# tatary/ramses

Hardware: AMD Instinct MI355X
Metric: cell-updates/s (Godunov sweep), uniform Sedov3D (higher is better)
Workload: dtype f64

## Files before the change

ramses_amd/csrc/hydro_core.hpp:

```cpp
#pragma once
#include <hip/hip_runtime.h>

namespace ramses_amd {

constexpr int RIEMANN_LLF = 0, RIEMANN_HLLC = 1, RIEMANN_HLL = 2,
              RIEMANN_ACOUSTIC = 3, RIEMANN_EXACT = 4;

constexpr int MAX_NENER = 2;
constexpr int MAX_NVAR = 16;

struct HydroConst {
  double gamma;
  double smallr;
  double smallc;
  double smallp;
  double smalle;
  double entho;
  double gm1;
  double smallc2;
  double gamma6;
  double smallpp;
  double oneovergamma;
  double slope_theta;
  int niter_riemann;
// ... 20 lines not shown
  r = __builtin_fma(r, e, r);
#endif
  return r;
}
RA_DEV double ddiv(double a, double b) { return a * rcp_fast(b); }
RA_DEV double dsqrt(double x) {
  double y = __builtin_amdgcn_rsq(x);
  double g = x * y;
  double h = 0.5 * y;
  double r = __builtin_fma(-h, g, 0.5);
  g = __builtin_fma(g, r, g);
  h = __builtin_fma(h, r, h);
  const double d = __builtin_fma(-g, g, x);
  g = __builtin_fma(d, h, g);
  return x == 0.0 ? 0.0 : g;
}
#else
RA_DEV double ddiv(double a, double b) { return a / b; }
RA_DEV double dsqrt(double x) { return __builtin_sqrt(x); }
#endif

template <int NV, bool GRAV, int NE = 0>
RA_DEV void ctoprim_cell(const double (&u)[NV], const double (&g)[3],
                         double dtxhalf, const HydroConst &P, double (&q)[NV]) {
  const double rho = dmaxd(u[0], P.smallr);
  const double oneoverrho = ddiv(1.0, rho);
  const double vx = u[1] * oneoverrho;
  const double vy = u[2] * oneoverrho;
  const double vz = u[3] * oneoverrho;
#ifdef RAMSES_AMD_FAST
  double k2 = vx * vx;
  k2 = __builtin_fma(vy, vy, k2);
  k2 = __builtin_fma(vz, vz, k2);
  double eint;
  if constexpr (NE == 0) {
    eint = dmaxd(__builtin_fma(u[4], oneoverrho, -0.5 * k2), P.smalle);
  } else {
    double erad = u[5] * oneoverrho;
    if constexpr (NE > 1) erad = __builtin_fma(u[6], oneoverrho, erad);
    eint = dmaxd(__builtin_fma(u[4], oneoverrho, -0.5 * k2) - erad, P.smalle);
  }
#else
  double eken = 0.5 * vx * vx;
  eken = eken + 0.5 * vy * vy;
  eken = eken + 0.5 * vz * vz;
  double eint;
  if constexpr (NE == 0) {
    eint = dmaxd(u[4] * oneoverrho - eken, P.smalle);
  } else {
// ... 104 lines not shown
  const double q0 = nb[13];
  double vmin = nb[0] - q0, vmax = vmin;
#pragma unroll
  for (int t = 1; t < 27; t++) {
    const double df = nb[t] - q0;
    vmin = dmind(vmin, df);
    vmax = dmaxd(vmax, df);
  }
  const double dfx = 0.5 * (nb[14] - nb[12]);
  const double dfy = 0.5 * (nb[16] - nb[10]);
  const double dfz = 0.5 * (nb[22] - nb[4]);
  const double dff = 0.5 * (__builtin_fabs(dfx) + __builtin_fabs(dfy) + __builtin_fabs(dfz));
  double slop = 1.0;
  if (dff > 0.0) slop = dmind(1.0, dmind(__builtin_fabs(vmin), __builtin_fabs(vmax)) / dff);
  d[0] = slop * dfx;
  d[1] = slop * dfy;
  d[2] = slop * dfz;
}

template <int NV, int NE = 0>
RA_DEV void trace3d_cell(const double (&q)[NV], const double (&dq)[3][NV],
                         double dtdx, double dtdy, double dtdz,
                         const HydroConst &P, double (&qm)[3][NV],
                         double (&qp)[3][NV]) {
  const double r = q[0], u = q[1], v = q[2], w = q[3], p = q[4];
  const double drx = dq[0][0], dux = dq[0][1], dvx = dq[0][2], dwx = dq[0][3], dpx = dq[0][4];
  const double dry = dq[1][0], duy = dq[1][1], dvy = dq[1][2], dwy = dq[1][3], dpy = dq[1][4];
  const double drz = dq[2][0], duz = dq[2][1], dvz = dq[2][2], dwz = dq[2][3], dpz = dq[2][4];
  const double div = dux + dvy + dwz;
#ifdef RAMSES_AMD_FAST
  const double rinv = rcp_fast(r);
  auto adv = [&](double ax, double ay, double az, double c0, double c1) {
    double t = u * ax;
    t = __builtin_fma(v, ay, t);
    t = __builtin_fma(w, az, t);
    return -__builtin_fma(c0, c1, t);
  };
  const double sr0 = adv(drx, dry, drz, div, r);
  const double sp0 = adv(dpx, dpy, dpz, div * P.gamma, p);
  double su0 = adv(dux, duy, duz, dpx, rinv);
  double sv0 = adv(dvx, dvy, dvz, dpy, rinv);
  double sw0 = adv(dwx, dwy, dwz, dpz, rinv);
  double se0[NE > 0 ? NE : 1];
#pragma unroll
  for (int i = 0; i < NE; i++) {
    su0 = __builtin_fma(-dq[0][5 + i], rinv, su0);
    sv0 = __builtin_fma(-dq[1][5 + i], rinv, sv0);
    sw0 = __builtin_fma(-dq[2][5 + i], rinv, sw0);
    se0[i] = adv(dq[0][5 + i], dq[1][5 + i], dq[2][5 + i], div * P.gamma_rad[i], q[5 + i]);
  }
#else
  const double sr0 = -u * drx - v * dry - w * drz - (div)*r;
  const double sp0 = -u * dpx - v * dpy - w * dpz - (div)*P.gamma * p;
  double su0 = -u * dux - v * duy - w * duz - (dpx) / r;
// ... 490 lines not shown
  a[2] = qL[4]; b[2] = qR[4];
  a[3] = qL[lt1]; b[3] = qR[lt1];
  a[4] = qL[lt2]; b[4] = qR[lt2];
#pragma unroll
  for (int n = 5; n < NV; n++) { a[n] = qL[n]; b[n] = qR[n]; }
  riemann_solve<RS, NV, NE>(a, b, P, f);
  flux[0] = f[0];
  flux[ln] = f[1];
  flux[lt1] = f[3];
  flux[lt2] = f[4];
  flux[4] = f[2];
#pragma unroll
  for (int n = 5; n < NV; n++) flux[n] = f[n];
  unorm = 0.5 * (a[1] + b[1]);
  eflux = f[NV];
}

#ifdef RAMSES_AMD_FAST
RA_DEV double rsqrt_fast(double x) {
  double y = __builtin_amdgcn_rsq(x);
  const double e = __builtin_fma(-(x * y), y, 1.0);
  return __builtin_fma(0.5 * y, e, y);
}
template <int DIR>
RA_DEV void llf_flux_fast(const double (&qL)[5], const double (&qR)[5],
                          const HydroConst &P, double dtdx, double (&flux)[5]) {
  constexpr int ln = DIR == 0 ? 1 : (DIR == 1 ? 2 : 3);
  constexpr int lt1 = DIR == 0 ? 2 : 1;
  constexpr int lt2 = DIR == 2 ? 2 : 3;
  const double rl = dmaxd(qL[0], P.smallr), pl = dmaxd(qL[4], rl * P.smallp);
  const double rr = dmaxd(qR[0], P.smallr), pr = dmaxd(qR[4], rr * P.smallp);
  const double gl = P.gamma * pl, gr = P.gamma * pr;
  const double cl = gl * rsqrt_fast(gl * rl);
  const double cr = gr * rsqrt_fast(gr * rr);
  const double ul = qL[ln], ur = qR[ln];
  const double cmax = dmaxd(__builtin_fabs(ul) + cl, __builtin_fabs(ur) + cr);
  const double hs = 0.5 * dtdx;
  const double hc = cmax * hs;
  const double mL = qL[0] * ul, mR = qR[0] * ur;
  double kL = ul * ul; kL = __builtin_fma(qL[lt1], qL[lt1], kL); kL = __builtin_fma(qL[lt2], qL[lt2], kL);
  double kR = ur * ur; kR = __builtin_fma(qR[lt1], qR[lt1], kR); kR = __builtin_fma(qR[lt2], qR[lt2], kR);
  const double eL = __builtin_fma(0.5 * qL[0], kL, qL[4] * P.entho);
  const double eR = __builtin_fma(0.5 * qR[0], kR, qR[4] * P.entho);
  const double t1L = qL[0] * qL[lt1], t1R = qR[0] * qR[lt1];
  const double t2L = qL[0] * qL[lt2], t2R = qR[0] * qR[lt2];
  const double fnL = __builtin_fma(ul, mL, qL[4]), fnR = __builtin_fma(ur, mR, qR[4]);
  const double feR = ur * (eR + qR[4]);
  const double fesum = __builtin_fma(ul, eL + qL[4], feR);
  flux[0] = __builtin_fma(hc, qL[0] - qR[0], hs * (mL + mR));
  flux[ln] = __builtin_fma(hc, mL - mR, hs * (fnL + fnR));
  flux[lt1] = __builtin_fma(hc, t1L - t1R, hs * __builtin_fma(ul, t1L, ur * t1R));
  flux[lt2] = __builtin_fma(hc, t2L - t2R, hs * __builtin_fma(ul, t2L, ur * t2R));
  flux[4] = __builtin_fma(hc, eL - eR, hs * fesum);
}
// ... 19 lines not shown
  const bool star = left ? !(SL > 0.0) : (SR > 0.0);
  const double rk = left ? rl : rr, uk = left ? ul : ur, Pk = left ? Pl : Pr, S = left ? SL : SR;
  const double vl1 = qL[lt1], vr1 = qR[lt1], vl2 = qL[lt2], vr2 = qR[lt2];
  const double w1 = left ? vl1 : vr1, w2 = left ? vl2 : vr2;
  double k2 = uk * uk; k2 = __builtin_fma(w1, w1, k2); k2 = __builtin_fma(w2, w2, k2);
  const double etk = __builtin_fma(0.5 * rk, k2, Pk * P.entho);
  const double inv = rcp_fast(S - ustar);
  const double dS = S - uk;
  const double rst = rk * dS * inv;
  const double ets = __builtin_fma(Pstar, ustar, __builtin_fma(dS, etk, -(Pk * uk))) * inv;
  const double ro = star ? rst : rk, uo = star ? ustar : uk, Po = star ? Pstar : Pk, eto = star ? ets : etk;
  const double m = ro * uo * dtdx;
  flux[0] = m;
  flux[ln] = __builtin_fma(m, uo, Po * dtdx);
  flux[lt1] = m * w1;
  flux[lt2] = m * w2;
  flux[4] = (eto + Po) * (uo * dtdx);
#if RAMSES_AMD_HLLC_FUSED == 2
  __builtin_amdgcn_sched_barrier(0);
#endif
}
#endif

template <int RS, int NV, int DIR, bool FUSE_HLLC = true, int NE = 0>
RA_DEV void scaled_interface_flux(const double (&qL)[NV], const double (&qR)[NV],
                                  const HydroConst &P, double dt, double dx, double rdx,
                                  double dtdx, bool DXPOW2, double (&flux)[NV]) {
#ifdef RAMSES_AMD_FAST
  if constexpr (RS == RIEMANN_LLF && NV == 5) {
    llf_flux_fast<DIR>(qL, qR, P, dtdx, flux);
    return;
  }
#ifndef RAMSES_AMD_HLLC_FUSED
#define RAMSES_AMD_HLLC_FUSED 1
#endif
  if constexpr (RAMSES_AMD_HLLC_FUSED != 0 && FUSE_HLLC && RS == RIEMANN_HLLC && NV == 5) {
    hllc_flux_fast<DIR>(qL, qR, P, dtdx, flux);
    return;
  }
#endif
  double un_, ef_;
  interface_flux<RS, NV, DIR, NE>(qL, qR, P, flux, un_, ef_);
#pragma unroll
  for (int n = 0; n < NV; n++) {
#ifdef RAMSES_AMD_FAST
    flux[n] = flux[n] * dtdx;
#else
    flux[n] = DXPOW2 ? flux[n] * dt * rdx : flux[n] * dt / dx;
#endif
  }
}

template <int RS, int NV, int DIR>
// ... 44 lines not shown
```

ramses_amd/csrc/hydro_sweep.hip:

```cpp
#include <hip/hip_runtime.h>

#include "hydro_core.hpp"
#include "sweep_args.hpp"

namespace ramses_amd {

#ifdef RAMSES_AMD_FAST
#define SWEEP_NS fastmode
#else
#define SWEEP_NS strictmode
#endif

namespace SWEEP_NS {

constexpr int BX = 64;
#ifndef TILE_SWEEP_BY
#define TILE_SWEEP_BY 12
#endif

template <int BY, int NV>
struct Plane {
  double v[NV][BY][BX];
};

template <int ST, int BY, int NV, bool MASK, bool GRAV, int NX = 0>
struct Lds {
  static constexpr int NF = NV + NX;
  static constexpr int RING = (ST == 3) ? 3 : 2;
#ifndef SWEEP_PARK_PLAIN
#ifdef RAMSES_AMD_FAST
#define SWEEP_PARK_PLAIN 1
#else
#define SWEEP_PARK_PLAIN 0
#endif
#endif
  static constexpr bool PARK = MASK || ((GRAV || SWEEP_PARK_PLAIN) && BY == 12);
  static constexpr int MR = PARK ? BY - 2 : BY;
  static constexpr int M0 = PARK ? 1 : 0;
  static constexpr size_t q_off = 0;
  static constexpr size_t m_off = q_off + RING * sizeof(Plane<BY, NV>);
  static constexpr size_t park_off = m_off + 2 * sizeof(Plane<MR, NF>);
  static constexpr size_t mask_off = park_off + (PARK ? sizeof(double) * 2 * NF * (BY - 4) * BX : 0);
  static constexpr size_t sloc_off = mask_off + (MASK ? 3 * BY * BX : 0);
  static constexpr size_t bytes = sloc_off + (MASK ? 4 * BY * BX : 0);
};

__device__ __forceinline__ double wave_shr1(double v) {
  int lo = __double2loint(v), hi = __double2hiint(v);
  lo = __builtin_amdgcn_update_dpp(lo, lo, 0x138, 0xf, 0xf, false);
  hi = __builtin_amdgcn_update_dpp(hi, hi, 0x138, 0xf, 0xf, false);
  return __hiloint2double(hi, lo);
}
__device__ __forceinline__ double wave_shl1(double v) {
  int lo = __double2loint(v), hi = __double2hiint(v);
  lo = __builtin_amdgcn_update_dpp(lo, lo, 0x130, 0xf, 0xf, false);
  hi = __builtin_amdgcn_update_dpp(hi, hi, 0x130, 0xf, 0xf, false);
  return __hiloint2double(hi, lo);
}

enum { ROLE_HALO = 0, ROLE_LOW = 1, ROLE_HIGH = 2, ROLE_FULL = 3, ROLE_HALO_HI = 4 };

typedef unsigned int v2u32 __attribute__((ext_vector_type(2)));
constexpr unsigned BUF_RANGE = 0x7fffffffu;
constexpr unsigned BUF_OOB = 0xffffffffu;
#ifndef SWEEP_STORE_AUX
#define SWEEP_STORE_AUX 0
#endif
__device__ __forceinline__ double plane_load(const double *var_base, unsigned plane_bytes, unsigned off) {
  __amdgpu_buffer_rsrc_t r = __builtin_amdgcn_make_buffer_rsrc(const_cast<double *>(var_base), 0, BUF_RANGE, 0x00020000);
  return __builtin_bit_cast(double, __builtin_amdgcn_raw_buffer_load_b64(r, off, plane_bytes, 0));
}
__device__ __forceinline__ void plane_store(double *var_base, unsigned plane_bytes, unsigned off, double x) {
  __amdgpu_buffer_rsrc_t r = __builtin_amdgcn_make_buffer_rsrc(var_base, 0, BUF_RANGE, 0x00020000);
  __builtin_amdgcn_raw_buffer_store_b64(__builtin_bit_cast(v2u32, x), r, off, plane_bytes, SWEEP_STORE_AUX);
}

__device__ __forceinline__ int wave_shr1_i(int v) { return __builtin_amdgcn_update_dpp(v, v, 0x138, 0xf, 0xf, false); }
__device__ __forceinline__ int wave_shl1_i(int v) { return __builtin_amdgcn_update_dpp(v, v, 0x130, 0xf, 0xf, false); }
__device__ __forceinline__ int stat_load(const unsigned char *base, unsigned ncell, unsigned lane_cell, unsigned plane_cell) {
  __amdgpu_buffer_rsrc_t r = __builtin_amdgcn_make_buffer_rsrc(const_cast<unsigned char *>(base), 0, ncell, 0x00020000);
  return (int)__builtin_amdgcn_raw_buffer_load_b8(r, lane_cell, plane_cell, 0);
}
__device__ __forceinline__ int dir_load(const int *base, unsigned plane_ints, unsigned col) {
  __amdgpu_buffer_rsrc_t r = __builtin_amdgcn_make_buffer_rsrc(const_cast<int *>(base), 0, BUF_RANGE, 0x00020000);
  return (int)__builtin_amdgcn_raw_buffer_load_b32(r, col * 4u, plane_ints * 4u, 0);
}

template <int ST, int RS, int BY, bool GRAV, int SCHEME, int NV, int ROLE, bool MASK, int NE = 0, bool PFIX = false>
__device__ __forceinline__ void sweep_march(const SweepArgs &A, unsigned char *smem_raw, const SweepPfix &X = SweepPfix()) {
  static_assert(!PFIX || (MASK && NE == 0 && SCHEME == 0), "pressure_fix: the sweep of a level in tiles, muscl");
  constexpr int NF = NV + (PFIX ? 2 : 0);
  const bool DXPOW2 = A.pow2 != 0;
  typedef Lds<ST, BY, NV, MASK, GRAV, NF - NV> L;
  constexpr int RING = L::RING;
  constexpr bool PARK = L::PARK;
  constexpr int M0 = L::M0;
  Plane<BY, NV> *qring = reinterpret_cast<Plane<BY, NV> *>(smem_raw + L::q_off);
  Plane<L::MR, NF> *mring = reinterpret_cast<Plane<L::MR, NF> *>(smem_raw + L::m_off);
  double (*park)[BY - 4][BX] = reinterpret_cast<double (*)[BY - 4][BX]>(smem_raw + L::park_off);

  const int tx = threadIdx.x, ty = threadIdx.y;
  const HydroConst &P = A.P;

  const int hb = blockIdx.x;
  int bi = 0;
#pragma unroll
  for (int i = 1; i < 6; i++)
    if (i < A.nbox && hb >= A.box[i].first) bi = i;
  const SweepBox &B = A.box[bi];
  int lb = hb - B.first;
  {
    const int nxcd = 8;
    const int cnt = (bi + 1 < A.nbox ? A.box[bi + 1].first : (int)gridDim.x) - B.first;
    if (cnt % nxcd == 0) {
      const int per = cnt / nxcd;
      lb = (lb % nxcd) * per + lb / nxcd;
    }
  }
#ifndef SWEEP_TILE_YFAST
#define SWEEP_TILE_YFAST 0
#endif
#if SWEEP_TILE_YFAST
// ... 47 lines not shown

#ifndef SWEEP_LATE_BASE
#define SWEEP_LATE_BASE 0
#endif
  constexpr bool LATE = SWEEP_LATE_BASE && NV == 5;
#ifndef SWEEP_KEEP_PLAIN
#define SWEEP_KEEP_PLAIN 1
#endif
#ifndef SWEEP_KEEP_STRICT
#define SWEEP_KEEP_STRICT 0
#endif
#if defined(RAMSES_AMD_FAST) || SWEEP_KEEP_STRICT
#ifndef SWEEP_KEEP_LLF_ONLY
#define SWEEP_KEEP_LLF_ONLY 0
#endif
#ifndef SWEEP_KEEP_NOT_HLLC
#define SWEEP_KEEP_NOT_HLLC 1
#endif
  constexpr bool KEEP = (MASK || (SWEEP_KEEP_PLAIN && BY == 12)) && NV == 5 && !LATE && (!SWEEP_KEEP_LLF_ONLY || RS == RIEMANN_LLF) &&
                        (!SWEEP_KEEP_NOT_HLLC || RS != RIEMANN_HLLC);
#else
  constexpr bool KEEP = false;
#endif
  constexpr bool r_trace = ROLE == ROLE_LOW || ROLE == ROLE_HIGH || ROLE == ROLE_FULL;
  constexpr bool r_fxz = ROLE == ROLE_FULL;
  const bool r_upd = r_fxz && (tx >= 2) && (tx <= BX - 3) && (xu < A.nx) && (yu < A.ny);
  const unsigned colb_upd = r_upd ? colb : BUF_OOB;

  const double dtdx = A.dt / A.dx;
  const double dtxhalf = A.dt * 0.5;

  auto plane_off = [&](int p) -> unsigned {
    int pz;
    if (A.ng == 0) { pz = p < 0 ? p + A.nz : (p >= A.nz ? p - A.nz : p); }
    else { pz = p + A.ng; }
    return (unsigned)pz * (unsigned)(A.pitch_z * 8);
  };
  auto wrap_z = [&](int p) -> int { return p < 0 ? p + A.nz : (p >= A.nz ? p - A.nz : p); };
  constexpr unsigned TILE_VOID = 0x80000000u;
  unsigned sA0 = TILE_VOID, sA1 = TILE_VOID, sB0 = TILE_VOID, sB1 = TILE_VOID;
  auto tile_of_plane = [&](int p) -> int { return wrap_z(p) >> 3; };
  auto tile_set = [&](int tz) {
    typedef const int __attribute__((address_space(4))) *cdir_p;
    const cdir_p row = (cdir_p)(A.dir + (long)tz * (A.ntx * A.nty) + drow);
    const int ra = row[tA], rb = row[tB];
    const unsigned a = ra < 0 ? TILE_VOID : (unsigned)ra * 8u, b = rb < 0 ? TILE_VOID : (unsigned)rb * 8u;
    if (tz & 1) { sA1 = a; sB1 = b; } else { sA0 = a; sB0 = b; }
  };
// ... 21 lines not shown
    if constexpr (PFIX) { u[NV] = plane_load(X.divu, pb, off); u[NV + 1] = plane_load(X.enew, pb, off); }
  };
  int ok_zlo = 0;
  int spre = 0;
  unsigned char *smask = smem_raw + L::mask_off;
  auto load_g = [&](int p, double (&g)[3]) {
    if (GRAV) {
      const unsigned pb = MASK ? zpart(p) * 8u : plane_off(p), off = MASK ? tbp(p) : colb;
#pragma unroll
      for (int d = 0; d < 3; d++) g[d] = plane_load(grav + (long)d * A.pitch_var, pb, off);
    } else {
      g[0] = g[1] = g[2] = 0.0;
    }
  };

  double qmz[NV];
  double fzlo[NF];
  double upre[NV], gpre[3];
  double rold = 0.0, sold[NV > 5 ? NV - 5 : 1];
  double ukeep[NV];
#pragma unroll
  for (int n = 0; n < NV; n++) ukeep[n] = 0.0;

  int sa = 0, sb = 1, sc = 2;

  if (MASK) {
    const int t0 = tile_of_plane(z0 - 2), t1 = t0 + 1 < A.ntz ? t0 + 1 : 0;
    tile_set(t0);
    tile_set(t1);
    __syncthreads();
    if (r_trace) spre = stat_load(A.stat, (unsigned)A.pitch_var, tbp(z0 - 1) >> 3, zpart(z0 - 1));
  }
  {
    double u[NV], g[3], q[NV];
    load_u(z0 - 2, u); load_g(z0 - 2, g);
    ctoprim_cell<NV, GRAV, NE>(u, g, dtxhalf, P, q);
#pragma unroll
    for (int n = 0; n < NV; n++) qring[sa].v[n][ty][tx] = q[n];
    load_u(z0 - 1, u); load_g(z0 - 1, g);
    if (KEEP) {
#pragma unroll
      for (int n = 0; n < NV; n++) ukeep[n] = u[n];
    }
    ctoprim_cell<NV, GRAV, NE>(u, g, dtxhalf, P, q);
#pragma unroll
    for (int n = 0; n < NV; n++) qring[sb].v[n][ty][tx] = q[n];
    load_u(z0, upre); load_g(z0, gpre);
#pragma unroll
    for (int n = 0; n < NV; n++) qmz[n] = 1.0;
#pragma unroll
    for (int n = 0; n < NF; n++) fzlo[n] = 0.0;
  }
  __builtin_amdgcn_s_waitcnt(0x0f70);
  __syncthreads();

  const int txm = tx - 1, txp = tx + 1;
  const int tym = ty - 1, typ = ty + 1;

  double partx[NF];
  double fyown[NF];
  double rnew = 0.0, snew[NV > 5 ? NV - 5 : 1];
  double bcar[NV];
#pragma unroll
  for (int n = 0; n < NV; n++) bcar[n] = 0.0;
#pragma unroll
  for (int n = 0; n < NF; n++) { partx[n] = 0.0; fyown[n] = 0.0; }
  if (PARK && r_fxz) {
#pragma unroll
    for (int n = 0; n < 2 * NF; n++) park[n][ty - 2][tx] = 0.0;
  }

  for (int c = z0 - 1; c <= z1; c++) {
    Plane<L::MR, NF> &M = mring[c & 1];
    Plane<L::MR, NF> &Mprev = mring[(c & 1) ^ 1];
    double qc[NV];
    ctoprim_cell<NV, GRAV, NE>(upre, gpre, dtxhalf, P, qc);
    if (RING == 3 || !r_trace) {
#pragma unroll
      for (int n = 0; n < NV; n++) qring[RING == 3 ? sc : sa].v[n][ty][tx] = qc[n];
    }
    double ucur[NF];
    if (r_fxz && !LATE) {
      if (KEEP && (!MASK || A.base_uold)) {
#pragma unroll
        for (int n = 0; n < NV; n++) ucur[n] = ukeep[n];
      } else if constexpr (MASK) load_base(c, ucur);
      else load_u(c, ucur);
    }
    if (KEEP && r_fxz) {
#pragma unroll
      for (int n = 0; n < NV; n++) ukeep[n] = upre[n];
    }
    int okc = 0, ok_ym = 0;
    if (MASK && r_trace) {
      okc = spre;
      smask[((c + 3) % 3 * BY + ty) * BX + tx] = (unsigned char)okc;
    }

    double qpy[NV], dz[NF], px[NF];
// ... 25 lines not shown
        for (int n = 0; n < NV; n++) qb[n] = qs.v[n][ty][tx];
        const double dc0 = qb[1] * A.dt / A.dx, dc1 = qb[2] * A.dt / A.dx, dc2 = qb[3] * A.dt / A.dx;
#pragma unroll
        for (int n = 0; n < NV; n++) {
          dq[0][n] = slope1_1d<ST>(qs.v[n][ty][txm], qb[n], qs.v[n][ty][txp], dc0, n);
          dq[1][n] = slope1_1d<ST>(qs.v[n][tym][tx], qb[n], qs.v[n][typ][tx], dc1, n);
          dq[2][n] = slope1_1d<ST>(qprev.v[n][ty][tx], qb[n], qc[n], dc2, n);
        }
      } else {
#pragma unroll
        for (int n = 0; n < NV; n++) {
          qb[n] = qs.v[n][ty][tx];
          dq[0][n] = slope1<ST>(qs.v[n][ty][txm], qb[n], qs.v[n][ty][txp], P);
          dq[1][n] = slope1<ST>(qs.v[n][tym][tx], qb[n], qs.v[n][typ][tx], P);
          dq[2][n] = slope1<ST>(qprev.v[n][ty][tx], qb[n], qc[n], P);
        }
      }
      if (RING == 2) {
#pragma unroll
        for (int n = 0; n < NV; n++) qring[sa].v[n][ty][tx] = qc[n];
      }
      double qm[3][NV], qp[3][NV];
      if (SCHEME == 0) {
        trace3d_cell<NV, NE>(qb, dq, dtdx, dtdx, dtdx, P, qm, qp);
      } else {
        const double cc = ctoprim_sound(qb[0], qb[4], P);
        tracexyz_cell<NV>(qb, dq, cc, dtdx, dtdx, dtdx, P, qm, qp);
      }
#pragma unroll
      for (int n = 0; n < NV; n++) M.v[n][ty - M0][tx] = qm[1][n];
#pragma unroll
      for (int n = 0; n < NV; n++) qpy[n] = qp[1][n];
      if constexpr (r_fxz) {
        double qL[NV], fx[NF], fz[NF];
#pragma unroll
        for (int n = 0; n < NV; n++) qL[n] = wave_shr1(qm[0][n]);
        if constexpr (PFIX) {
          double f[NV], t[2];
          scaled_interface_flux_tmp<RS, NV, 0>(qL, qp[0], P, A.dt, A.dx, A.rdx, DXPOW2, f, t);
#pragma unroll
          for (int n = 0; n < NV; n++) fx[n] = f[n];
          fx[NV] = t[0]; fx[NV + 1] = t[1];
          scaled_interface_flux_tmp<RS, NV, 2>(qmz, qp[2], P, A.dt, A.dx, A.rdx, DXPOW2, f, t);
#pragma unroll
          for (int n = 0; n < NV; n++) fz[n] = f[n];
          fz[NV] = t[0]; fz[NV + 1] = t[1];
        } else {
        scaled_interface_flux<RS, NV, 0, !MASK, NE>(qL, qp[0], P, A.dt, A.dx, A.rdx, dtdx, DXPOW2, fx);
        scaled_interface_flux<RS, NV, 2, !MASK, NE>(qmz, qp[2], P, A.dt, A.dx, A.rdx, dtdx, DXPOW2, fz);
        }
        if (MASK) {
          const int s_xm = wave_shr1_i(okc);
          const bool zx = ((okc | s_xm) & CELL_REFINED) != 0, zz = ((okc | ok_zlo) & CELL_REFINED) != 0;
#pragma unroll
          for (int n = 0; n < NF; n++) { fx[n] = zx ? 0.0 : fx[n]; fz[n] = zz ? 0.0 : fz[n]; }
        }
        double fxh[NF];
#pragma unroll
        for (int n = 0; n < NV; n++) qmz[n] = qm[2][n];
#pragma unroll
        for (int n = 0; n < NF; n++) {
          dz[n] = fzlo[n] - fz[n];
          fzlo[n] = fz[n];
          fxh[n] = wave_shl1(fx[n]);
          px[n] = LATE ? (fx[n] - fxh[n]) : ucur[n] + (fx[n] - fxh[n]);
        }
        if (NV > 5 + NE && !MASK) {
          rnew = ucur[0];
#pragma unroll
          for (int n = 5 + NE; n < NV; n++) snew[n - 5] = ucur[n];
        }
      }
    }
    __builtin_amdgcn_sched_barrier(0);
    {
      const int pn = min(c + 2, z1 + 1);
      if (MASK) {
        const int lp = wrap_z(pn) & 7;
        const int tn = tile_of_plane(pn) + 1 < A.ntz ? tile_of_plane(pn) + 1 : 0;
        if (lp == 4) tile_set(tn);
      }
      load_u(pn, upre); load_g(pn, gpre);
      if (MASK && r_trace) { const int ps = min(c + 1, z1 + 1); spre = stat_load(A.stat, (unsigned)A.pitch_var, tbp(ps) >> 3, zpart(ps)); }
    }
    __builtin_amdgcn_sched_barrier(0);
    __syncthreads();

    double fy[NF];
    if constexpr (ROLE == ROLE_FULL || ROLE == ROLE_HIGH) {
      double qL[NV];
#pragma unroll
      for (int n = 0; n < NV; n++) qL[n] = M.v[n][tym - M0][tx];
      if constexpr (PFIX) {
        double f[NV], t[2];
        scaled_interface_flux_tmp<RS, NV, 1>(qL, qpy, P, A.dt, A.dx, A.rdx, DXPOW2, f, t);
#pragma unroll
        for (int n = 0; n < NV; n++) fy[n] = f[n];
        fy[NV] = t[0]; fy[NV + 1] = t[1];
      } else {
      scaled_interface_flux<RS, NV, 1, !MASK, NE>(qL, qpy, P, A.dt, A.dx, A.rdx, dtdx, DXPOW2, fy);
      }
      if (MASK) {
        ok_ym = smask[((c + 3) % 3 * BY + tym) * BX + tx];
        const bool zy = ((okc | ok_ym) & CELL_REFINED) != 0;
#pragma unroll
        for (int n = 0; n < NF; n++) fy[n] = zy ? 0.0 : fy[n];
      }
#pragma unroll
      for (int n = 0; n < NF; n++) M.v[n][tym - M0][tx] = fy[n];
    }
    if constexpr (r_fxz) {
      double un[NF], fyh[NF];
#pragma unroll
      for (int n = 0; n < NF; n++) {
        fyh[n] = Mprev.v[n][ty - M0][tx];
        const double pxn = PARK ? park[n][ty - 2][tx] : partx[n];
        const double fyn = PARK ? park[NF + n][ty - 2][tx] : fyown[n];
        const double part = (LATE ? bcar[n < NV ? n : 0] + pxn : pxn) + (fyn - fyh[n]);
        un[n] = part + dz[n];
      }
      if (NV > 5 + NE && !MASK) {
        if (rold < P.smallr && un[0] > rold) {
#pragma unroll
          for (int n = 5 + NE; n < NV; n++) un[n] = sold[n - 5] * dmaxd(un[0], P.smallr) / P.smallr;
        } else if (un[0] < P.smallr && rold > un[0]) {
#pragma unroll
          for (int n = 5 + NE; n < NV; n++) un[n] = sold[n - 5] * P.smallr / dmaxd(rold, P.smallr);
        }
        rold = rnew;
#pragma unroll
        for (int n = 5 + NE; n < NV; n++) sold[n - 5] = snew[n - 5];
      }
#pragma unroll
      for (int n = 0; n < NF; n++) {
        if (PARK) { park[n][ty - 2][tx] = px[n]; park[NF + n][ty - 2][tx] = fy[n]; }
        else { partx[n] = px[n]; fyown[n] = fy[n]; }
      }
      {
        const unsigned pb = MASK ? zpart(c - 1) * 8u : plane_off(c - 1);
        const unsigned so = (c >= z0 + 1) ? (MASK ? ((r_upd && (ok_zlo & CELL_OWNED)) ? tbp(c - 1) : BUF_OOB) : colb_upd) : BUF_OOB;
#pragma unroll
        for (int n = 0; n < NV; n++) {
          if (MASK) plane_store(unew + (long)(n & ~1) * A.pitch_var, pb + (n & 1) * odd_var, so, un[n]);
          else plane_store(unew + (long)n * A.pitch_var, pb, so, un[n]);
        }
        if constexpr (PFIX) { plane_store(X.divu, pb, so, un[NV]); plane_store(X.enew, pb, so, un[NV + 1]); }
      }
      if constexpr (LATE) { if (MASK) load_base(c, bcar); else load_u(c, bcar); }
    }
    if (RING == 3) { const int t = sa; sa = sb; sb = sc; sc = t; }
    else { const int t = sa; sa = sb; sb = t; }
    if (MASK) ok_zlo = okc;
  }
}

template <int ST, int RS, int BY, bool GRAV, int SCHEME, int NV, bool MASK = false>
__global__ __launch_bounds__(BX *BY) void godunov_sweep_kernel(SweepArgs A) {
  extern __shared__ __attribute__((aligned(16))) unsigned char smem_raw[];
  const int ty = threadIdx.y;
  if (ty >= 2 && ty <= BY - 3) __builtin_amdgcn_s_setprio(3);
  if (ty == 0) sweep_march<ST, RS, BY, GRAV, SCHEME, NV, ROLE_HALO, MASK>(A, smem_raw);
  else if (ty == BY - 1) sweep_march<ST, RS, BY, GRAV, SCHEME, NV, ROLE_HALO_HI, MASK>(A, smem_raw);
  else if (ty == 1) sweep_march<ST, RS, BY, GRAV, SCHEME, NV, ROLE_LOW, MASK>(A, smem_raw);
  else if (ty == BY - 2) sweep_march<ST, RS, BY, GRAV, SCHEME, NV, ROLE_HIGH, MASK>(A, smem_raw);
  else sweep_march<ST, RS, BY, GRAV, SCHEME, NV, ROLE_FULL, MASK>(A, smem_raw);
}

#ifndef RAMSES_AMD_FAST
template <int ST, int NV>
struct PfixRows {
  static constexpr int BY = (ST == 3 && NV == 7) ? 6 : 8;
};
template <int ST, int RS, int BY, bool GRAV, int NV>
__global__ __launch_bounds__(BX *BY) void godunov_sweep_pfix_kernel(SweepArgs A, SweepPfix X) {
  extern __shared__ __attribute__((aligned(16))) unsigned char smem_raw[];
  static_assert(Lds<ST, BY, NV, true, GRAV, 2>::bytes <= 160 * 1024, "the pressure_fix sweep fits one workgroup's LDS");
  const int ty = threadIdx.y;
  if (ty >= 2 && ty <= BY - 3) __builtin_amdgcn_s_setprio(3);
  if (ty == 0) sweep_march<ST, RS, BY, GRAV, 0, NV, ROLE_HALO, true, 0, true>(A, smem_raw, X);
  else if (ty == BY - 1) sweep_march<ST, RS, BY, GRAV, 0, NV, ROLE_HALO_HI, true, 0, true>(A, smem_raw, X);
  else if (ty == 1) sweep_march<ST, RS, BY, GRAV, 0, NV, ROLE_LOW, true, 0, true>(A, smem_raw, X);
  else if (ty == BY - 2) sweep_march<ST, RS, BY, GRAV, 0, NV, ROLE_HIGH, true, 0, true>(A, smem_raw, X);
  else sweep_march<ST, RS, BY, GRAV, 0, NV, ROLE_FULL, true, 0, true>(A, smem_raw, X);
}
#endif

template <int ST, int RS, int NV, int NE>
__global__ __launch_bounds__(BX * 8) void godunov_sweep_nener_kernel(SweepArgs A) {
// ... 522 lines not shown
  }
  return hipErrorInvalidValue;
}
#ifndef RAMSES_AMD_FAST
hipError_t launch_surface_flux_pfix(const SurfArgs &A, int slope_type, int riemann, int nvar, bool grav, hipStream_t s) {
  if (A.nevent <= 0) return hipSuccess;
  switch (slope_type) {
    case 1: return surface0_pfix<1>(A, riemann, nvar, grav, s);
#ifndef SWEEP_FLAGSHIP_ONLY
    case 0: return surface0_pfix<0>(A, riemann, nvar, grav, s);
    case 2: return surface0_pfix<2>(A, riemann, nvar, grav, s);
    case 3: return surface0_pfix<3>(A, riemann, nvar, grav, s);
    case 7: return surface0_pfix<7>(A, riemann, nvar, grav, s);
    case 8: return surface0_pfix<8>(A, riemann, nvar, grav, s);
#endif
  }
  return hipErrorInvalidValue;
}
#endif
#endif

template <int ST, int RS, int BY, bool GRAV, int SCHEME, int NV, bool MASK = false>
static hipError_t launch3(const SweepArgs &A, hipStream_t s) {
  const size_t lds = Lds<ST, BY, NV, MASK, GRAV>::bytes;
  dim3 block(BX, BY);
  dim3 grid(A.nblocks);
  auto k = godunov_sweep_kernel<ST, RS, BY, GRAV, SCHEME, NV, MASK>;
  hipError_t e = hipFuncSetAttribute(reinterpret_cast<const void *>(k), hipFuncAttributeMaxDynamicSharedMemorySize, (int)lds);
  if (e != hipSuccess) return e;
  hipLaunchKernelGGL(k, grid, block, lds, s, A);
  return hipGetLastError();
}

template <int ST, int RS, int BY, int SCHEME, int NV>
static hipError_t launch2(const SweepArgs &A, bool grav, hipStream_t s) {
  return grav ? launch3<ST, RS, BY, true, SCHEME, NV>(A, s) : launch3<ST, RS, BY, false, SCHEME, NV>(A, s);
}

static int plan_boxes(SweepArgs &A, int by) {
  const int NTX = (A.nx + (BX - 4) - 1) / (BX - 4);
  const int NTY = (A.ny + (by - 4) - 1) / (by - 4);
  const int zb = 2;
  const bool splittable = NTX >= 3 && NTY >= 3 && A.nz >= 4 * zb;
  A.nbox = 0;
  int nblocks = 0;
  auto add_box = [&](int tx0, int tx1, int ty0, int ty1, int zlo, int zhi, int zchunk) {
    if (tx1 <= tx0 || ty1 <= ty0 || zhi <= zlo) return;
// ... 323 lines not shown
}

hipError_t launch_godunov_sweep_scalars(SweepArgs &A, int slope_type, int riemann, int by, int nvar, int nener, bool grav, hipStream_t s) {
  if ((unsigned long)A.pitch_z * 8ul >= (1ul << 31) || (unsigned long)A.pitch_var * 8ul >= (1ul << 32))
    return hipErrorInvalidValue;
  switch (slope_type) {
    case 1: return launch0_scalar<1>(A, riemann, by, nvar, nener, grav, s);
#ifndef SWEEP_FLAGSHIP_ONLY
    case 0: return launch0_scalar<0>(A, riemann, by, nvar, nener, grav, s);
    case 2: return launch0_scalar<2>(A, riemann, by, nvar, nener, grav, s);
    case 3: return launch0_scalar<3>(A, riemann, by, nvar, nener, grav, s);
    case 7: return launch0_scalar<7>(A, riemann, by, nvar, nener, grav, s);
    case 8: return launch0_scalar<8>(A, riemann, by, nvar, nener, grav, s);
#endif
  }
  return hipErrorInvalidValue;
}

#endif

}
}

#include "warm.hpp"
#if defined(SWEEP_ST)
#elif RAMSES_AMD_FAST
RAMSES_AMD_TU_WARM(hydro_sweep_fast)
#else
RAMSES_AMD_TU_WARM(hydro_sweep_strict)
#endif
```

Before: 45.20 billion.

## Reuse density reciprocal in trace, skip redundant floors, add y-flux duty sharing

In fast mode with LLF, the 1/rho computed in ctoprim is carried to the next iteration and reused in trace3d instead of a second reciprocal. The interface flux also skips the smallr floor, since densities are already floored. A y-flux work redistribution (behind SWEEP_YDUTY, off by default) moves some row-2 and row BY-2 y-flux computations onto the halo rows through a new LDS buffer. A cycle-counter probe, also off by default, is added too. The reuse adds a register carried across loop iterations and assumes trace inputs are already floored.

```diff
diff --git a/ramses_amd/csrc/hydro_core.hpp b/ramses_amd/csrc/hydro_core.hpp
--- a/ramses_amd/csrc/hydro_core.hpp
+++ b/ramses_amd/csrc/hydro_core.hpp
@@ -66,9 +66,10 @@
 
 template <int NV, bool GRAV, int NE = 0>
 RA_DEV void ctoprim_cell(const double (&u)[NV], const double (&g)[3],
-                         double dtxhalf, const HydroConst &P, double (&q)[NV]) {
+                         double dtxhalf, const HydroConst &P, double (&q)[NV], double *rinv_out = nullptr) {
   const double rho = dmaxd(u[0], P.smallr);
   const double oneoverrho = ddiv(1.0, rho);
+  if (rinv_out) *rinv_out = oneoverrho;
   const double vx = u[1] * oneoverrho;
   const double vy = u[2] * oneoverrho;
   const double vz = u[3] * oneoverrho;
@@ -219,14 +220,14 @@
 RA_DEV void trace3d_cell(const double (&q)[NV], const double (&dq)[3][NV],
                          double dtdx, double dtdy, double dtdz,
                          const HydroConst &P, double (&qm)[3][NV],
-                         double (&qp)[3][NV]) {
+                         double (&qp)[3][NV], const double *rinv_in = nullptr) {
   const double r = q[0], u = q[1], v = q[2], w = q[3], p = q[4];
   const double drx = dq[0][0], dux = dq[0][1], dvx = dq[0][2], dwx = dq[0][3], dpx = dq[0][4];
   const double dry = dq[1][0], duy = dq[1][1], dvy = dq[1][2], dwy = dq[1][3], dpy = dq[1][4];
   const double drz = dq[2][0], duz = dq[2][1], dvz = dq[2][2], dwz = dq[2][3], dpz = dq[2][4];
   const double div = dux + dvy + dwz;
 #ifdef RAMSES_AMD_FAST
-  const double rinv = rcp_fast(r);
+  const double rinv = rinv_in ? *rinv_in : rcp_fast(r);
   auto adv = [&](double ax, double ay, double az, double c0, double c1) {
     double t = u * ax;
     t = __builtin_fma(v, ay, t);
@@ -763,14 +764,14 @@
   const double e = __builtin_fma(-(x * y), y, 1.0);
   return __builtin_fma(0.5 * y, e, y);
 }
-template <int DIR>
+template <int DIR, bool FLOORED = false>
 RA_DEV void llf_flux_fast(const double (&qL)[5], const double (&qR)[5],
                           const HydroConst &P, double dtdx, double (&flux)[5]) {
   constexpr int ln = DIR == 0 ? 1 : (DIR == 1 ? 2 : 3);
   constexpr int lt1 = DIR == 0 ? 2 : 1;
   constexpr int lt2 = DIR == 2 ? 2 : 3;
-  const double rl = dmaxd(qL[0], P.smallr), pl = dmaxd(qL[4], rl * P.smallp);
-  const double rr = dmaxd(qR[0], P.smallr), pr = dmaxd(qR[4], rr * P.smallp);
+  const double rl = FLOORED ? qL[0] : dmaxd(qL[0], P.smallr), pl = dmaxd(qL[4], rl * P.smallp);
+  const double rr = FLOORED ? qR[0] : dmaxd(qR[0], P.smallr), pr = dmaxd(qR[4], rr * P.smallp);
   const double gl = P.gamma * pl, gr = P.gamma * pr;
   const double cl = gl * rsqrt_fast(gl * rl);
   const double cr = gr * rsqrt_fast(gr * rr);
@@ -836,13 +837,13 @@
 }
 #endif
 
-template <int RS, int NV, int DIR, bool FUSE_HLLC = true, int NE = 0>
+template <int RS, int NV, int DIR, bool FUSE_HLLC = true, int NE = 0, bool FLOORED = false>
 RA_DEV void scaled_interface_flux(const double (&qL)[NV], const double (&qR)[NV],
                                   const HydroConst &P, double dt, double dx, double rdx,
                                   double dtdx, bool DXPOW2, double (&flux)[NV]) {
 #ifdef RAMSES_AMD_FAST
   if constexpr (RS == RIEMANN_LLF && NV == 5) {
-    llf_flux_fast<DIR>(qL, qR, P, dtdx, flux);
+    llf_flux_fast<DIR, FLOORED>(qL, qR, P, dtdx, flux);
     return;
   }
 #ifndef RAMSES_AMD_HLLC_FUSED
diff --git a/ramses_amd/csrc/hydro_sweep.hip b/ramses_amd/csrc/hydro_sweep.hip
--- a/ramses_amd/csrc/hydro_sweep.hip
+++ b/ramses_amd/csrc/hydro_sweep.hip
@@ -23,7 +23,7 @@
   double v[NV][BY][BX];
 };
 
-template <int ST, int BY, int NV, bool MASK, bool GRAV, int NX = 0>
+template <int ST, int BY, int NV, bool MASK, bool GRAV, int NX = 0, bool DUTY = false>
 struct Lds {
   static constexpr int NF = NV + NX;
   static constexpr int RING = (ST == 3) ? 3 : 2;
@@ -40,7 +40,8 @@
   static constexpr size_t q_off = 0;
   static constexpr size_t m_off = q_off + RING * sizeof(Plane<BY, NV>);
   static constexpr size_t park_off = m_off + 2 * sizeof(Plane<MR, NF>);
-  static constexpr size_t mask_off = park_off + (PARK ? sizeof(double) * 2 * NF * (BY - 4) * BX : 0);
+  static constexpr size_t duty_off = park_off + (PARK ? sizeof(double) * 2 * NF * (BY - 4) * BX : 0);
+  static constexpr size_t mask_off = duty_off + (DUTY ? sizeof(double) * 2 * NF * BX : 0);
   static constexpr size_t sloc_off = mask_off + (MASK ? 3 * BY * BX : 0);
   static constexpr size_t bytes = sloc_off + (MASK ? 4 * BY * BX : 0);
 };
@@ -58,7 +59,33 @@
   return __hiloint2double(hi, lo);
 }
 
-enum { ROLE_HALO = 0, ROLE_LOW = 1, ROLE_HIGH = 2, ROLE_FULL = 3, ROLE_HALO_HI = 4 };
+enum { ROLE_HALO = 0, ROLE_LOW = 1, ROLE_HIGH = 2, ROLE_FULL = 3, ROLE_HALO_HI = 4, ROLE_FULL_LO = 5 };
+
+#ifndef SWEEP_YDUTY
+#define SWEEP_YDUTY 0
+#endif
+template <int ST, int RS, int BY, bool GRAV, int SCHEME, int NV, bool MASK, int NE = 0, bool PFIX = false>
+constexpr bool y_duty() {
+  return SWEEP_YDUTY && SWEEP_PARK_PLAIN && RS == RIEMANN_LLF && BY == 12 && ST != 3 && !GRAV && SCHEME == 0 && NV == 5 && !MASK && NE == 0 && !PFIX;
+}
+template <int BY, bool DUTY>
+constexpr int yflux_wave(int f) { return !DUTY ? f : (f == 2 ? 0 : (f == BY - 2 ? BY - 1 : f)); }
+
+#ifndef SWEEP_TRIM
+#ifdef RAMSES_AMD_FAST
+#define SWEEP_TRIM 1
+#else
+#define SWEEP_TRIM 0
+#endif
+#endif
+
+#ifndef SWEEP_CYCLE_PROBE
+#define SWEEP_CYCLE_PROBE 0
+#endif
+#if SWEEP_CYCLE_PROBE
+constexpr int PROBE_BLOCKS = 8192, PROBE_ROWS = 12, PROBE_WORDS = 6;
+static __device__ unsigned long long sweep_cycle_probe[PROBE_BLOCKS][PROBE_ROWS][PROBE_WORDS];
+#endif
 
 typedef unsigned int v2u32 __attribute__((ext_vector_type(2)));
 constexpr unsigned BUF_RANGE = 0x7fffffffu;
@@ -91,13 +118,16 @@
   static_assert(!PFIX || (MASK && NE == 0 && SCHEME == 0), "pressure_fix: the sweep of a level in tiles, muscl");
   constexpr int NF = NV + (PFIX ? 2 : 0);
   const bool DXPOW2 = A.pow2 != 0;
-  typedef Lds<ST, BY, NV, MASK, GRAV, NF - NV> L;
+  constexpr bool DUTY = y_duty<ST, RS, BY, GRAV, SCHEME, NV, MASK, NE, PFIX>();
+  static_assert(DUTY || ROLE != ROLE_FULL_LO, "row 2 is a full row like the others unless the y fluxes are shared out");
+  typedef Lds<ST, BY, NV, MASK, GRAV, NF - NV, DUTY> L;
   constexpr int RING = L::RING;
   constexpr bool PARK = L::PARK;
   constexpr int M0 = L::M0;
   Plane<BY, NV> *qring = reinterpret_cast<Plane<BY, NV> *>(smem_raw + L::q_off);
   Plane<L::MR, NF> *mring = reinterpret_cast<Plane<L::MR, NF> *>(smem_raw + L::m_off);
   double (*park)[BY - 4][BX] = reinterpret_cast<double (*)[BY - 4][BX]>(smem_raw + L::park_off);
+  double (*yduty)[NF][BX] = reinterpret_cast<double (*)[NF][BX]>(smem_raw + L::duty_off);
 
   const int tx = threadIdx.x, ty = threadIdx.y;
   const HydroConst &P = A.P;
@@ -191,8 +221,14 @@
 #else
   constexpr bool KEEP = false;
 #endif
-  constexpr bool r_trace = ROLE == ROLE_LOW || ROLE == ROLE_HIGH || ROLE == ROLE_FULL;
-  constexpr bool r_fxz = ROLE == ROLE_FULL;
+  constexpr bool r_fxz = ROLE == ROLE_FULL || ROLE == ROLE_FULL_LO;
+  constexpr bool r_trace = ROLE == ROLE_LOW || ROLE == ROLE_HIGH || r_fxz;
+  constexpr bool y_give = DUTY && (ROLE == ROLE_FULL_LO || ROLE == ROLE_HIGH);
+  constexpr bool y_take = DUTY && (ROLE == ROLE_HALO || ROLE == ROLE_HALO_HI);
+  constexpr int DUTY_F = ROLE == ROLE_HALO ? 2 : BY - 2;
+  static_assert(!DUTY || (yflux_wave<BY, DUTY>(2) == 0 && yflux_wave<BY, DUTY>(BY - 2) == BY - 1 && yflux_wave<BY, DUTY>(3) == 3),
+                "the roles below implement this table");
+  constexpr bool TRIM = SWEEP_TRIM != 0 && RS == RIEMANN_LLF && SCHEME == 0 && NE == 0 && !PFIX;
   const bool r_upd = r_fxz && (tx >= 2) && (tx <= BX - 3) && (xu < A.nx) && (yu < A.ny);
   const unsigned colb_upd = r_upd ? colb : BUF_OOB;
 
@@ -260,6 +296,11 @@
 #pragma unroll
   for (int n = 0; n < NV; n++) ukeep[n] = 0.0;
 
+  double rinv_c = 0.0;
+#if SWEEP_CYCLE_PROBE
+  unsigned long long pr_a = 0, pr_w = 0, pr_b = 0, pr_n = 0;
+#endif
+
   int sa = 0, sb = 1, sc = 2;
 
   if (MASK) {
@@ -280,7 +321,8 @@
 #pragma unroll
       for (int n = 0; n < NV; n++) ukeep[n] = u[n];
     }
-    ctoprim_cell<NV, GRAV, NE>(u, g, dtxhalf, P, q);
+    if constexpr (TRIM && r_trace) ctoprim_cell<NV, GRAV, NE>(u, g, dtxhalf, P, q, &rinv_c);
+    else ctoprim_cell<NV, GRAV, NE>(u, g, dtxhalf, P, q);
 #pragma unroll
     for (int n = 0; n < NV; n++) qring[sb].v[n][ty][tx] = q[n];
     load_u(z0, upre); load_g(z0, gpre);
@@ -307,12 +349,21 @@
 #pragma unroll
     for (int n = 0; n < 2 * NF; n++) park[n][ty - 2][tx] = 0.0;
   }
+  if constexpr (DUTY && ROLE == ROLE_FULL_LO) {
+#pragma unroll
+    for (int n = 0; n < NF; n++) yduty[0][n][tx] = yduty[1][n][tx] = 0.0;
+  }
 
   for (int c = z0 - 1; c <= z1; c++) {
     Plane<L::MR, NF> &M = mring[c & 1];
     Plane<L::MR, NF> &Mprev = mring[(c & 1) ^ 1];
+#if SWEEP_CYCLE_PROBE
+    const unsigned long long pr_t0 = __builtin_readcyclecounter();
+#endif
     double qc[NV];
-    ctoprim_cell<NV, GRAV, NE>(upre, gpre, dtxhalf, P, qc);
+    double rinv_n = 0.0;
+    if constexpr (TRIM && r_trace) ctoprim_cell<NV, GRAV, NE>(upre, gpre, dtxhalf, P, qc, &rinv_n);
+    else ctoprim_cell<NV, GRAV, NE>(upre, gpre, dtxhalf, P, qc);
     if (RING == 3 || !r_trace) {
 #pragma unroll
       for (int n = 0; n < NV; n++) qring[RING == 3 ? sc : sa].v[n][ty][tx] = qc[n];
@@ -384,15 +435,20 @@
       }
       double qm[3][NV], qp[3][NV];
       if (SCHEME == 0) {
-        trace3d_cell<NV, NE>(qb, dq, dtdx, dtdx, dtdx, P, qm, qp);
+        if constexpr (TRIM) trace3d_cell<NV, NE>(qb, dq, dtdx, dtdx, dtdx, P, qm, qp, &rinv_c);
+        else trace3d_cell<NV, NE>(qb, dq, dtdx, dtdx, dtdx, P, qm, qp);
       } else {
         const double cc = ctoprim_sound(qb[0], qb[4], P);
         tracexyz_cell<NV>(qb, dq, cc, dtdx, dtdx, dtdx, P, qm, qp);
       }
 #pragma unroll
-      for (int n = 0; n < NV; n++) M.v[n][ty - M0][tx] = qm[1][n];
+      for (int n = 0; n < NV; n++) M.v[n][ty - M0][tx] = (DUTY && ROLE == ROLE_HIGH) ? qp[1][n] : qm[1][n];
 #pragma unroll
       for (int n = 0; n < NV; n++) qpy[n] = qp[1][n];
+      if constexpr (DUTY && ROLE == ROLE_FULL_LO) {
+#pragma unroll
+        for (int n = 0; n < NV; n++) yduty[c & 1][n][tx] = qp[1][n];
+      }
       if constexpr (r_fxz) {
         double qL[NV], fx[NF], fz[NF];
 #pragma unroll
@@ -408,8 +464,8 @@
           for (int n = 0; n < NV; n++) fz[n] = f[n];
           fz[NV] = t[0]; fz[NV + 1] = t[1];
         } else {
-        scaled_interface_flux<RS, NV, 0, !MASK, NE>(qL, qp[0], P, A.dt, A.dx, A.rdx, dtdx, DXPOW2, fx);
-        scaled_interface_flux<RS, NV, 2, !MASK, NE>(qmz, qp[2], P, A.dt, A.dx, A.rdx, dtdx, DXPOW2, fz);
+        scaled_interface_flux<RS, NV, 0, !MASK, NE, TRIM>(qL, qp[0], P, A.dt, A.dx, A.rdx, dtdx, DXPOW2, fx);
+        scaled_interface_flux<RS, NV, 2, !MASK, NE, TRIM>(qmz, qp[2], P, A.dt, A.dx, A.rdx, dtdx, DXPOW2, fz);
         }
         if (MASK) {
           const int s_xm = wave_shr1_i(okc);
@@ -446,10 +502,30 @@
       if (MASK && r_trace) { const int ps = min(c + 1, z1 + 1); spre = stat_load(A.stat, (unsigned)A.pitch_var, tbp(ps) >> 3, zpart(ps)); }
     }
     __builtin_amdgcn_sched_barrier(0);
+#if SWEEP_CYCLE_PROBE
+    const unsigned long long pr_t1 = __builtin_readcyclecounter();
+#endif
     __syncthreads();
+#if SWEEP_CYCLE_PROBE
+    const unsigned long long pr_t2 = __builtin_readcyclecounter();
+#endif
 
     double fy[NF];
-    if constexpr (ROLE == ROLE_FULL || ROLE == ROLE_HIGH) {
+    if constexpr (y_take) {
+      double qL[NV], qR[NV];
+#pragma unroll
+      for (int n = 0; n < NV; n++) {
+        qL[n] = M.v[n][DUTY_F - 1 - M0][tx];
+        qR[n] = ROLE == ROLE_HALO ? yduty[c & 1][n][tx] : M.v[n][DUTY_F - M0][tx];
+      }
+      scaled_interface_flux<RS, NV, 1, !MASK, NE, TRIM>(qL, qR, P, A.dt, A.dx, A.rdx, dtdx, DXPOW2, fy);
+#pragma unroll
+      for (int n = 0; n < NF; n++) {
+        if (ROLE == ROLE_HALO) yduty[c & 1][n][tx] = fy[n];
+        else M.v[n][DUTY_F - 1 - M0][tx] = fy[n];
+      }
+    }
+    if constexpr ((r_fxz || ROLE == ROLE_HIGH) && !y_give) {
       double qL[NV];
 #pragma unroll
       for (int n = 0; n < NV; n++) qL[n] = M.v[n][tym - M0][tx];
@@ -460,7 +536,7 @@
         for (int n = 0; n < NV; n++) fy[n] = f[n];
         fy[NV] = t[0]; fy[NV + 1] = t[1];
       } else {
-      scaled_interface_flux<RS, NV, 1, !MASK, NE>(qL, qpy, P, A.dt, A.dx, A.rdx, dtdx, DXPOW2, fy);
+      scaled_interface_flux<RS, NV, 1, !MASK, NE, TRIM>(qL, qpy, P, A.dt, A.dx, A.rdx, dtdx, DXPOW2, fy);
       }
       if (MASK) {
         ok_ym = smask[((c + 3) % 3 * BY + tym) * BX + tx];
@@ -477,7 +553,7 @@
       for (int n = 0; n < NF; n++) {
         fyh[n] = Mprev.v[n][ty - M0][tx];
         const double pxn = PARK ? park[n][ty - 2][tx] : partx[n];
-        const double fyn = PARK ? park[NF + n][ty - 2][tx] : fyown[n];
+        const double fyn = y_give ? yduty[(c & 1) ^ 1][n][tx] : (PARK ? park[NF + n][ty - 2][tx] : fyown[n]);
         const double part = (LATE ? bcar[n < NV ? n : 0] + pxn : pxn) + (fyn - fyh[n]);
         un[n] = part + dz[n];
       }
@@ -495,7 +571,7 @@
       }
 #pragma unroll
       for (int n = 0; n < NF; n++) {
-        if (PARK) { park[n][ty - 2][tx] = px[n]; park[NF + n][ty - 2][tx] = fy[n]; }
+        if (PARK) { park[n][ty - 2][tx] = px[n]; if (!y_give) park[NF + n][ty - 2][tx] = fy[n]; }
         else { partx[n] = px[n]; fyown[n] = fy[n]; }
       }
       {
@@ -513,7 +589,18 @@
     if (RING == 3) { const int t = sa; sa = sb; sb = sc; sc = t; }
     else { const int t = sa; sa = sb; sb = t; }
     if (MASK) ok_zlo = okc;
-  }
+    if (TRIM) rinv_c = rinv_n;
+#if SWEEP_CYCLE_PROBE
+    pr_a += pr_t1 - pr_t0; pr_w += pr_t2 - pr_t1; pr_b += __builtin_readcyclecounter() - pr_t2; pr_n += 1;
+#endif
+  }
+#if SWEEP_CYCLE_PROBE
+  if (tx == 0 && blockIdx.x < PROBE_BLOCKS && ty < PROBE_ROWS) {
+    unsigned long long *o = sweep_cycle_probe[blockIdx.x][ty];
+    o[0] = pr_a; o[1] = pr_w; o[2] = pr_b; o[3] = pr_n; o[4] = (unsigned long long)ty;
+    o[5] = (unsigned long long)__builtin_amdgcn_s_getreg((31 << 11) | 4);
+  }
+#endif
 }
 
 template <int ST, int RS, int BY, bool GRAV, int SCHEME, int NV, bool MASK = false>
@@ -525,7 +612,12 @@
   else if (ty == BY - 1) sweep_march<ST, RS, BY, GRAV, SCHEME, NV, ROLE_HALO_HI, MASK>(A, smem_raw);
   else if (ty == 1) sweep_march<ST, RS, BY, GRAV, SCHEME, NV, ROLE_LOW, MASK>(A, smem_raw);
   else if (ty == BY - 2) sweep_march<ST, RS, BY, GRAV, SCHEME, NV, ROLE_HIGH, MASK>(A, smem_raw);
-  else sweep_march<ST, RS, BY, GRAV, SCHEME, NV, ROLE_FULL, MASK>(A, smem_raw);
+  else {
+    if constexpr (y_duty<ST, RS, BY, GRAV, SCHEME, NV, MASK>()) {
+      if (ty == 2) { sweep_march<ST, RS, BY, GRAV, SCHEME, NV, ROLE_FULL_LO, MASK>(A, smem_raw); return; }
+    }
+    sweep_march<ST, RS, BY, GRAV, SCHEME, NV, ROLE_FULL, MASK>(A, smem_raw);
+  }
 }
 
 #ifndef RAMSES_AMD_FAST
@@ -1094,7 +1186,9 @@
 
 template <int ST, int RS, int BY, bool GRAV, int SCHEME, int NV, bool MASK = false>
 static hipError_t launch3(const SweepArgs &A, hipStream_t s) {
-  const size_t lds = Lds<ST, BY, NV, MASK, GRAV>::bytes;
+  typedef Lds<ST, BY, NV, MASK, GRAV, 0, y_duty<ST, RS, BY, GRAV, SCHEME, NV, MASK>()> L;
+  static_assert(L::bytes <= 160 * 1024, "one workgroup's LDS");
+  const size_t lds = L::bytes;
   dim3 block(BX, BY);
   dim3 grid(A.nblocks);
   auto k = godunov_sweep_kernel<ST, RS, BY, GRAV, SCHEME, NV, MASK>;
@@ -1464,6 +1558,16 @@
 }
 }
 
+#if SWEEP_CYCLE_PROBE && defined(RAMSES_AMD_FAST) && defined(SWEEP_ST) && SWEEP_ST == 1
+extern "C" int ramses_amd_sweep_cycle_probe(unsigned long long *out, long nwords) {
+  using namespace ramses_amd::fastmode;
+  const long have = (long)PROBE_BLOCKS * PROBE_ROWS * PROBE_WORDS;
+  if (hipDeviceSynchronize() != hipSuccess) return -1;
+  if (hipMemcpyFromSymbol(out, HIP_SYMBOL(sweep_cycle_probe), sizeof(unsigned long long) * (nwords < have ? nwords : have)) != hipSuccess) return -1;
+  return 0;
+}
+#endif
+
 #include "warm.hpp"
 #if defined(SWEEP_ST)
 #elif RAMSES_AMD_FAST
```

Result: faster. 45.80 billion, median of 6 (+1.3%).
